# bodono/scs-python

Measured on AMD Instinct MI355X. Metric: ADMM iters/sec (random LP+SOC cone program, indirect CG linsys, AA lookback 10), higher is better.
Workload: dtype f64; 1 GPU; target_lp_soc: m=2000000 n=1000000 nnz=19999909 cone={'l': 1000000, 'q': '100000x10'} seed=5(+rank); one independent instance per GPU; world_size_seen=1

## Files before the change

### include/scs_hip.h

```cpp
#ifndef SCS_HIP_H_GUARD
#define SCS_HIP_H_GUARD

#include "scs_types.h"

#ifdef __cplusplus
extern "C" {
#endif

#define SCS_HIP_API __attribute__((visibility("default")))

typedef struct ScsHipWork ScsWork;


SCS_HIP_API ScsWork *scs_init(const ScsData *d, const ScsCone *k, const ScsSettings *stgs);

SCS_HIP_API scs_int scs_solve(ScsWork *w, ScsSolution *sol, ScsInfo *info, scs_int warm_start);

SCS_HIP_API scs_int scs_update(ScsWork *w, scs_float *b, scs_float *c);

SCS_HIP_API void scs_finish(ScsWork *w);

SCS_HIP_API void scs_set_default_settings(ScsSettings *stgs);

SCS_HIP_API const char *scs_version(void);
// ... 21 lines not shown

SCS_HIP_API int scs_hip_grad_matrix_sum(scs_int m, scs_int n, const scs_int *Ap, const scs_int *Ai, const scs_int *Pp, const scs_int *Pi, scs_int K,
                                        const scs_float *X, const scs_float *Y, const scs_float *DB, const scs_float *DC, scs_float *out_dA,
                                        scs_float *out_dP);

SCS_HIP_API int scs_hip_proj_cone_seq(scs_float *xs, const ScsCone *k, scs_int m, int dual, int count, scs_float *stats, int stats_cap);

SCS_HIP_API int scs_hip_kkt_solve(const ScsMatrix *A, const ScsMatrix *P, const scs_float *diag_r, scs_float *rhs,
                      scs_float tol, scs_int *cg_iters);

SCS_HIP_API int scs_hip_kkt_solve_dense(const ScsMatrix *A, const ScsMatrix *P, const scs_float *diag_r, scs_float *rhs);

SCS_HIP_API ScsWork *scs_hip_init_linsys(const ScsData *d, const ScsCone *k, const ScsSettings *stgs, int linsys);
SCS_HIP_API int scs_hip_linsys_kind(const ScsWork *w);

SCS_HIP_API int scs_hip_normalize(ScsMatrix *A, ScsMatrix *P, scs_float *b, scs_float *c, const ScsCone *k,
                      scs_float *D, scs_float *E, scs_float *sigma);

SCS_HIP_API double scs_hip_copy_bandwidth(size_t bytes, int reps);

SCS_HIP_API void scs_hip_set_profiling(ScsWork *w, int on);
SCS_HIP_API void scs_hip_kernel_times(const ScsWork *w, double *out);
SCS_HIP_API int scs_hip_solution_to_device(ScsWork *w, scs_float *x_dev, scs_float *y_dev, scs_float *s_dev);

SCS_HIP_API scs_int scs_hip_update_device(ScsWork *w, const scs_float *b_dev, const scs_float *c_dev);
SCS_HIP_API scs_int scs_hip_solve_device(ScsWork *w, scs_float *x_dev, scs_float *y_dev, scs_float *s_dev, ScsInfo *info, scs_int warm_start);
SCS_HIP_API scs_int scs_hip_solve_batch_device(ScsWork **w, scs_float **x_dev, scs_float **y_dev, scs_float **s_dev, ScsInfo **info,
                                               scs_int count, scs_int warm_start);
SCS_HIP_API scs_int scs_hip_update_matrix(ScsWork *w, const scs_float *Ax, const scs_float *Px);
SCS_HIP_API scs_int scs_hip_update_matrix_device(ScsWork *w, const scs_float *Ax_dev, const scs_float *Px_dev);
typedef struct {
  scs_float tol;
  scs_int max_iters;
} ScsHipDiffOpts;
typedef struct {
  scs_int iters;
  scs_float residual, normal_residual;
  scs_int stop;
  scs_float time_ms;
} ScsHipDiffInfo;
SCS_HIP_API scs_int scs_hip_adjoint_device(ScsWork *w, const scs_float *gx_dev, const scs_float *gy_dev, const scs_float *gs_dev,
                                           scs_float *db_dev, scs_float *dc_dev, scs_float *dAx_dev, scs_float *dPx_dev,
                                           const ScsHipDiffOpts *opts, ScsHipDiffInfo *info);
SCS_HIP_API scs_int scs_hip_adjoint(ScsWork *w, const scs_float *gx, const scs_float *gy, const scs_float *gs, scs_float *db, scs_float *dc,
                                    scs_float *dAx, scs_float *dPx, const ScsHipDiffOpts *opts, ScsHipDiffInfo *info);
SCS_HIP_API scs_int scs_hip_derivative_device(ScsWork *w, const scs_float *db_dev, const scs_float *dc_dev, scs_float *dx_dev,
// ... 96 lines not shown
```

### scs-python_amd/csrc/loop.hpp

```cpp
#pragma once
static void fill_nan(double *p, long nelem) {
  for (long i = 0; i < nelem; ++i) p[i] = NAN;
}

struct InterruptListener {
  static std::atomic<int> &flag() { static std::atomic<int> f{0}; return f; }
  static void on_sigint(int) { flag().store(1, std::memory_order_relaxed); }
  static bool enabled() { static const bool on = [] { const char *e = getenv("SCS_HIP_CTRLC"); return !(e && e[0] == '0'); }(); return on; }
  static std::mutex &mtx() { static std::mutex m; return m; }
  static int &users() { static int u = 0; return u; }
  static struct sigaction &saved() { static struct sigaction sa; return sa; }
  InterruptListener() {
    if (!enabled()) return;
    std::lock_guard<std::mutex> g(mtx());
    if (users()++ == 0) {
      flag().store(0);
      struct sigaction sa;
      std::memset(&sa, 0, sizeof(sa));
      sa.sa_handler = on_sigint;
      sigemptyset(&sa.sa_mask);
      sa.sa_flags = SA_RESTART;
      sigaction(SIGINT, &sa, &saved());
    }
  }
  ~InterruptListener() {
    if (!enabled()) return;
    std::lock_guard<std::mutex> g(mtx());
    if (--users() == 0) {
      struct sigaction cur;
      if (sigaction(SIGINT, nullptr, &cur) == 0 && cur.sa_handler == on_sigint) sigaction(SIGINT, &saved(), nullptr);
    }
  }
  static bool interrupted() { return enabled() && flag().load(std::memory_order_relaxed) != 0; }
};

static scs_int solve_impl(ScsHipWork *w, ScsSolution *sol, ScsInfo *info, scs_int warm_start, bool dev_io = false) {
  std::lock_guard<std::mutex> lock(w->mtx);
  InterruptListener ctrlc;
  HIP_CHECK(hipSetDevice(w->device));
  ScsHipWork::ScratchTurn turn(w);
  const int n = w->n, m = w->m;
  const long l = w->l;
  hipStream_t s = w->stream;
  w->finish_pending_setup();
  const double t_start = now_ms();
  w->begin_solve(sol, info, warm_start, dev_io);
  double t_lin = 0, t_cone = 0, t_acc = 0;
  FILE *csv = nullptr;
  if (!w->log_csv_filename.empty()) {
    csv = std::fopen(w->log_csv_filename.c_str(), "w");
    if (csv) std::fputs(kCsvHeader, csv);
  }
  const bool verbose = w->stgs.verbose != 0;
  if (verbose) {
    std::printf("------------------------------------------------------------------\n");
    std::printf("\t  scs-hip v%s - MI355X-native Splitting Conic Solver path\n", scs_version());
    std::printf("------------------------------------------------------------------\n");
    std::printf("problem:  variables n: %d, constraints m: %d\n", n, m);
    std::printf("cones: \t  z: %d, l: %d, box: %d, q: %zu, s: %zu, cs: %zu, ep: %d, ed: %d, p: %zu\n", w->cone.z, w->cone.l,
                w->cone.bsize, w->cone.q.size(), w->cone.s.size(), w->cone.cs.size(), w->cone.ep, w->cone.ed,
                w->cone.p.size());
    if (w->cone.has_spectral())
      std::printf("\t  d: %zu, nuc: %zu, ell1: %zu, sl: %zu\n", w->cone.d.size(), w->cone.nuc_m.size(), w->cone.ell1.size(),
                  w->cone.sl_n.size());
    std::printf("settings: eps_abs: %.1e, eps_rel: %.1e, eps_infeas: %.1e\n\t  alpha: %.2f, scale: %.2e, adaptive_scale: %d\n"
                "\t  max_iters: %d, normalize: %d, rho_x: %.2e\n\t  acceleration_lookback: %d, acceleration_interval: %d\n",
                w->stgs.eps_abs, w->stgs.eps_rel, w->stgs.eps_infeas, w->stgs.alpha, w->scale, w->stgs.adaptive_scale,
                w->stgs.max_iters, w->stgs.normalize, w->stgs.rho_x, w->stgs.acceleration_lookback,
                w->stgs.acceleration_interval);
// ... 78 lines not shown
      w->populate_residuals(i);
      std::printf("%6d|%9.2e|%9.2e|%9.2e|%9.2e|%9.2e|%9.2e\n", i, w->r.res_pri, w->r.res_dual, w->r.gap,
                  0.5 * (w->r.pobj + w->r.dobj), w->scale, (now_ms() - t_start) / 1e3);
      std::fflush(stdout);
    }
    if (w->stgs.adaptive_scale && check && i == w->r.last_iter) w->update_scale(i);
    w->enqueue_v_update();
    if (csv) w->log_csv_row(csv, i, now_ms() - t_start);
    if (aa_now) {
      t = now_ms();
      w->aa_safeguard();
      t_acc += now_ms() - t;
    }
  }
  if (csv) std::fclose(csv);
  if (w->debug_pipe()) {
    std::fprintf(stderr, "[scs-hip] iterations %d, run-ahead stalls %d, CG steps of the last 8 solves:", i, w->pipe_stalls);
    for (int v : w->cg_hist) std::fprintf(stderr, " %d", v);
    std::fprintf(stderr, "\n");
  }
  w->finish_solve(sol, info, i, t_start, t_lin, t_cone, t_acc, false, dev_io);
  std::vector<double> foot;
  ScsSolution foot_sol{nullptr, nullptr, nullptr};
  if (verbose && dev_io) {
    foot.resize(2 * (size_t)m);
    foot_sol.y = foot.data();
    foot_sol.s = foot.data() + m;
    w->soly.download(foot_sol.y, m, s);
    w->sols.download(foot_sol.s, m, s);
    HIP_CHECK(hipStreamSynchronize(s));
    sol = &foot_sol;
  }
  if (verbose) {
    std::printf("------------------------------------------------------------------\n");
    std::printf("status:  %s\ntimings: total: %.2es = setup: %.2es + solve: %.2es\n\t lin-sys: %.2es, cones: %.2es, accel: %.2es\n",
                info->status, (info->setup_time + info->solve_time) / 1e3, info->setup_time / 1e3, info->solve_time / 1e3,
                t_lin / 1e3, t_cone / 1e3, t_acc / 1e3);
    std::printf("lin-sys: avg cg its: %.2f\n", info->iter > 0 ? (double)w->tot_cg_iters / (info->iter + 1) : 0.0);
    std::printf("------------------------------------------------------------------\n");
    switch (info->status_val) {
      case SCS_SOLVED:
      case SCS_SOLVED_INACCURATE: {
        double sy = 0., ns = 0., ny = 0.;
        for (int j = 0; j < m; ++j) { sy += sol->s[j] * sol->y[j]; ns += sol->s[j] * sol->s[j]; ny += sol->y[j] * sol->y[j]; }
        std::printf("cones: dist(s, K) = %.2e, dist(y, K*) = %.2e\n", w->cone_dist(sol->s, 0), w->cone_dist(sol->y, 1));
        std::printf("comp slack: s'y/|s||y| = %.2e, gap: |x'Px+c'x+b'y| = %.2e\n", safediv_pos(sy, std::sqrt(ns) * std::sqrt(ny)), info->gap);
        std::printf("pri res: |Ax+s-b| = %.2e, dua res: |Px+A'y+c| = %.2e\n", info->res_pri, info->res_dual);
// ... 21 lines not shown
```

### scs-python_amd/csrc/options.hpp

```cpp
#pragma once
#include <atomic>
#include <cstdlib>
#include <cstring>
#include <mutex>
#include <string>

extern char **environ;

namespace scship {

enum : unsigned { DBG_PIPE = 1u, DBG_GROUP = 2u, DBG_SETUP = 4u, DBG_TOL = 8u };

struct Options {
  bool pipeline = true;
  int pipe_chunk = 0;
  bool host_setup = false;
  bool lazy_setup = true;
  bool cs = true;
  long cs_min_nnz = 1L << 20;
  bool cs_split = true;
  bool slab = true;
  bool aa_gram = false;
  int psd_split = -1;
  int psd_mc = -1;
  bool psd_refine = true;
  bool psd_tol_adaptive = true;
  int spin_budget_log2 = 25;
  bool linsys_dense = false;
  unsigned debug = 0;

  bool psd_coop = false;
  bool cs_combine = false;
  int cs_rpt = 0, cs_split_a = 0, cs_split_at = 0;
  bool cs_peel = true, cs_virt = true;
// ... 13 lines not shown
      o.pipe_chunk = v >= 2 ? v : 0;
    }
    if (const char *e = getenv("SCS_HIP_SETUP")) o.host_setup = e[0] == 'h';
    o.lazy_setup = !is0(getenv("SCS_HIP_LAZY_SETUP"));
    if (const char *e = getenv("SCS_HIP_CS")) {
      const long v = atol(e);
      o.cs = !is0(e);
      if (v >= 2) o.cs_min_nnz = v;
    }
    o.cs_split = !is0(getenv("SCS_HIP_CS_SPLIT"));
    o.slab = !is0(getenv("SCS_HIP_SLAB"));
    if (const char *e = getenv("SCS_HIP_AA")) o.aa_gram = e[0] == 'g';
    if (const char *e = getenv("SCS_HIP_PSD_SPLIT")) o.psd_split = e[0] == '1' ? 1 : 0;
    if (const char *e = getenv("SCS_HIP_PSD_MC")) o.psd_mc = atoi(e);
    o.psd_refine = !is0(getenv("SCS_HIP_PSD_REFINE"));
    if (const char *e = getenv("SCS_HIP_PSD_TOL")) o.psd_tol_adaptive = e[0] != 'f';
    if (const char *e = getenv("SCS_HIP_SPIN_BUDGET_LOG2")) { const int v = atoi(e); o.spin_budget_log2 = v < 0 ? 0 : (v > 40 ? 40 : v); }
    if (const char *e = getenv("SCS_HIP_LINSYS")) o.linsys_dense = e[0] == 'd' || e[0] == 'D';
    if (const char *e = getenv("SCS_HIP_DEBUG")) {
      if (strstr(e, "pipe")) o.debug |= DBG_PIPE;
      if (strstr(e, "group")) o.debug |= DBG_GROUP;
      if (strstr(e, "setup")) o.debug |= DBG_SETUP;
      if (strstr(e, "tol")) o.debug |= DBG_TOL;
      if (strstr(e, "all")) o.debug = ~0u;
    }
#ifdef SCS_HIP_LABS
    auto pos_int = [](const char *name, int dflt) { const char *e = getenv(name); const int v = e ? atoi(e) : 0; return v > 0 ? v : dflt; };
    auto pos_dbl = [](const char *name, double dflt) { const char *e = getenv(name); const double v = e ? atof(e) : 0.; return v > 0. ? v : dflt; };
    o.psd_coop = is1(getenv("SCS_HIP_PSD_COOP"));
    o.cs_combine = is1(getenv("SCS_HIP_CS_COMBINE"));
    { const int v = pos_int("SCS_HIP_CS_RPT", 0); o.cs_rpt = (v == 1 || v == 2 || v == 4 || v == 8 || v == 16) ? v : 0; }
    o.cs_split_a = pos_int("SCS_HIP_CS_SPLIT_A", 0);
    o.cs_split_at = pos_int("SCS_HIP_CS_SPLIT_AT", 0);
    o.cs_peel = !is0(getenv("SCS_HIP_CS_PEEL"));
    o.cs_virt = !is0(getenv("SCS_HIP_CS_VIRT"));
    o.cg_fuse = !is0(getenv("SCS_HIP_CG_FUSE"));
    o.norm_fuse = !is0(getenv("SCS_HIP_NORM_FUSE"));
    o.soc_psd_fuse = !is0(getenv("SCS_HIP_SOC_PSD_FUSE"));
    o.psd_tol_k = pos_dbl("SCS_HIP_PSD_TOL_K", 1e-2);
    o.psd_la = !is0(getenv("SCS_HIP_PSD_LA"));
    o.psd_mc_nocheck = getenv("SCS_HIP_PSD_MC_NOCHECK") != nullptr;
    o.pool_poison = is1(getenv("SCS_HIP_POOL_POISON"));
    if (const char *e = getenv("SCS_HIP_SHARED_TILE")) o.shared_tile = e[0] != '0';
#endif
    return o;
  }
// ... 27 lines not shown
```

### scs-python_amd/csrc/scs_hip.hip

```cpp
#include <atomic>
#include <cstddef>
#include <chrono>
#include <csignal>
#include <functional>
#include <memory>
#include <mutex>
#include <thread>

#include "options.hpp"
#include "aa.hpp"
#include "common.hpp"
#include "cones.hpp"
#include "host_setup.hpp"
#include "normalize_dev.hpp"
#include "psd.hpp"
#include "spectral.hpp"
#include "dense.hpp"
#include "setup_dev.hpp"
#include "setup_cs_dev.hpp"
#include "spmv.hpp"
#include "vec.hpp"
#include "device_io.hpp"
#include "dproj.hpp"
#include "lsqr.hpp"

#include "runtime.hpp"
#include "device_csr.hpp"
#include "work.hpp"
#include "io.hpp"
#include "setup.hpp"
#include "loop.hpp"
#include "batch.hpp"
#include "matrix_update.hpp"
#include "perturb.hpp"
#include "diff.hpp"
#include "diff_batch.hpp"
#include "grad_shared.hpp"

static ScsCone short_cone(const ScsCone *k) {
  ScsCone c;
  std::memset(&c, 0, sizeof(c));
  if (k) std::memcpy(&c, k, offsetof(ScsCone, d));
  return c;
}

extern "C" {

ScsWork *scs_init(const ScsData *d, const ScsCone *k, const ScsSettings *stgs) {
  try {
// ... 28 lines not shown
}

ScsWork *scs_hip_init_linsys_spectral(const ScsData *d, const ScsCone *k, const ScsSettings *stgs, int linsys) {
  try {
    set_last_error("");
    return init_impl(d, k, stgs, linsys);
  } catch (const std::exception &e) {
    set_last_error(e.what());
    return nullptr;
  }
}
ScsWork *scs_hip_clone(ScsWork *w) {
  try {
    set_last_error("");
    return clone_impl(w);
  } catch (const std::exception &e) {
    set_last_error(e.what());
    return nullptr;
  }
}
int scs_hip_shares_matrix(const ScsWork *a, const ScsWork *b) { return a && b && a->mats == b->mats ? 1 : 0; }
int scs_hip_linsys_kind(const ScsWork *w) { return w ? (w->dense() ? 2 : 1) : 0; }

static void fill_failed(ScsHipWork *w, ScsSolution *sol, bool dev_io) {
  if (!dev_io) {
    fill_nan(sol->x, w->n);
    fill_nan(sol->y, w->m);
    fill_nan(sol->s, w->m);
    return;
  }
  if (hipSetDevice(w->device) != hipSuccess) return;
  const double *ptr[3] = {sol->x, sol->y, sol->s};
  const long len[3] = {w->n, w->m, w->m};
  for (int k = 0; k < 3; ++k)
    if (ptr[k]) hipLaunchKernelGGL(k_fill, dim3(vec_blocks(len[k])), dim3(kVecThreads), 0, w->stream, (double *)ptr[k], (double)NAN, len[k]);
  (void)hipStreamSynchronize(w->stream);
  (void)hipGetLastError();
}

static scs_int solve_entry(ScsWork *w, ScsSolution *sol, ScsInfo *info, scs_int warm_start, bool dev_io) {
  try {
    set_last_error("");
    const double scale_entry = w->scale;
    try {
      return solve_impl(w, sol, info, warm_start, dev_io);
    } catch (const SpinTimeout &) {
      ++g_spin_fallbacks;
      {
        std::lock_guard<std::mutex> lock(w->mtx);
        HIP_CHECK(hipSetDevice(w->device));
        w->spin_fallback(scale_entry);
      }
      return solve_impl(w, sol, info, warm_start, dev_io);
    }
  } catch (const std::exception &e) {
    set_last_error(e.what());
    info->status_val = SCS_FAILED;
    std::snprintf(info->status, sizeof(info->status), "failure");
    fill_failed(w, sol, dev_io);
    return SCS_FAILED;
  }
}

scs_int scs_solve(ScsWork *w, ScsSolution *sol, ScsInfo *info, scs_int warm_start) {
  if (!w || !sol || !info) return SCS_FAILED;
  return solve_entry(w, sol, info, warm_start, false);
}

static void check_device_vector(const void *p, int device, const char *who, const char *name) {
  hipPointerAttribute_t a;
  std::memset(&a, 0, sizeof(a));
  const hipError_t e = hipPointerGetAttributes(&a, p);
  if (e != hipSuccess) (void)hipGetLastError();
  if (e != hipSuccess || a.type != hipMemoryTypeDevice)
    throw std::runtime_error(std::string(who) + ": " + name + " is not a device address");
  if (a.device != device)
    throw std::runtime_error(std::string(who) + ": " + name + " lives on device " + std::to_string(a.device) + ", the workspace on device " +
                             std::to_string(device));
}
static void check_device_solution(const ScsHipWork *w, const double *x, const double *y, const double *s, scs_int warm_start, const char *who) {
  if (warm_start && (!x || !y || !s)) throw std::runtime_error(std::string(who) + ": a warm start needs x_dev, y_dev and s_dev");
  if (x) check_device_vector(x, w->device, who, "x_dev");
  if (y) check_device_vector(y, w->device, who, "y_dev");
  if (s) check_device_vector(s, w->device, who, "s_dev");
}

scs_int scs_hip_update_device(ScsWork *w, const scs_float *b_dev, const scs_float *c_dev) {
  if (!w) return -1;
  try {
// ... 2 lines not shown
    if (c_dev) check_device_vector(c_dev, w->device, "scs_hip_update_device", "c_dev");
    std::lock_guard<std::mutex> lock(w->mtx);
    HIP_CHECK(hipSetDevice(w->device));
    ScsHipWork::ScratchTurn turn(w);
    w->diff_mark_stale();
    w->update_device(b_dev, c_dev);
    return 0;
  } catch (const std::exception &e) {
    set_last_error(e.what());
    return -1;
  }
}

scs_int scs_hip_solve_device(ScsWork *w, scs_float *x_dev, scs_float *y_dev, scs_float *s_dev, ScsInfo *info, scs_int warm_start) {
  if (!w || !info) return -1;
  try {
    set_last_error("");
    check_device_solution(w, x_dev, y_dev, s_dev, warm_start, "scs_hip_solve_device");
  } catch (const std::exception &e) {
    set_last_error(e.what());
    return -1;
  }
  ScsSolution sol{x_dev, y_dev, s_dev};
  return solve_entry(w, &sol, info, warm_start, true);
}
int scs_hip_work_device(const ScsWork *w) { return w ? w->device : -1; }

static scs_int solve_one_group(ScsWork **works, ScsSolution **sols, ScsInfo **infos, const std::vector<int> &idx, scs_int warm_start,
                               std::string &err, bool dev_io, const Options &o) {
  if (idx.size() == 1) {
    const int i = idx[0];
    const scs_int st = solve_entry(works[i], sols[i], infos[i], warm_start, dev_io);
    if (st == SCS_FAILED) { err = scs_hip_last_error(); return -1; }
    return 0;
  }
  scs_int rc = 0;
  std::vector<std::unique_lock<std::mutex>> locks;
  std::vector<hipStream_t> saved;
  GroupSolve gs(o);
  for (int j : idx) {
    std::memset(infos[j], 0, sizeof(ScsInfo));
    infos[j]->status_val = SCS_UNFINISHED;
  }
  try {
    {
      std::vector<int> order(idx);
      std::sort(order.begin(), order.end(), [&](int a, int b) { return std::less<ScsHipWork *>()(works[a], works[b]); });
      for (int j : order) locks.emplace_back(works[j]->mtx);
    }
    HIP_CHECK(hipSetDevice(works[idx[0]]->device));
    gs.s = works[idx[0]]->stream;
    gs.dev_io = dev_io;
    for (int j : idx) {
      gs.W.push_back(works[j]); gs.sols.push_back(sols[j]); gs.infos.push_back(infos[j]);
      saved.push_back(works[j]->stream);
// ... 910 lines not shown
```

### scs-python_amd/csrc/work.hpp

```cpp
#pragma once
using namespace scship;

static void write_csv_row(FILE *f, int iter, const Residuals &r, double scale, const double *diffs, double aa_norm,
                          double time_s);

struct SpinTimeout : std::runtime_error {
  using std::runtime_error::runtime_error;
};
static std::atomic<long> g_spin_fallbacks{0};
struct SpinChain {
  std::mutex mu;
  int users = 0;
  hipEvent_t last = nullptr;
  hipStream_t last_stream = nullptr;
};
static SpinChain &spin_chain(int device) {
  static SpinChain c[64];
  return c[device & 63];
}

struct MatrixSet {
  const Options &opt;
  explicit MatrixSet(const Options &o) : opt(o) {}
  std::shared_ptr<Arena> home;
// ... 68 lines not shown

  DeviceCsr &At = mats->At;
  DeviceCsr &Ar = mats->Ar;
  DeviceCsr &Pf = mats->Pf;
  DevBuf<double> &Pdiag = mats->Pdiag;
  DevBuf<double> &D = mats->D, &E = mats->E;

  DevBuf<double> v, v_prev, u, ut, rsk, g, h, diag_r, Dinv, Einv;
  DevBuf<double> cg_b, cg_p, cg_r, cg_Gp, cg_M, tmp_m, ws, px;
  DevBuf<double> part, part2, sc, out;
  DevBuf<double> part_v;
  bool v_norm_fresh = false;
  DevBuf<int> fl;
  DevBuf<double> solx, soly, sols;
  bool sol_on_device = false;
  int diff_state = 0, last_status_val = 0;
  void diff_mark_stale() { if (diff_state == 1) diff_state = 3; }
  DiffScratch diff;
  DevBuf<double> b_raw, c_raw;
  DevBuf<unsigned> io_ticket;
  bool b_raw_fresh = false, c_raw_fresh = false, b_host_stale = false, c_host_stale = false;
  double *sol_pin = nullptr;
  bool sol_pin_refused = false;
  hipEvent_t sol_ev[3] = {nullptr, nullptr, nullptr};
  static constexpr size_t kSolMirrorMin = (size_t)1 << 20;
  static void spread_memcpy(void *dst, const void *src, size_t bytes) {
    const int nt = bytes >= ((size_t)8 << 20) ? 4 : 1;
    if (nt == 1) { std::memcpy(dst, src, bytes); return; }
    const size_t part = (bytes / nt + 4095) & ~(size_t)4095;
    std::thread th[3];
    for (int t = 1; t < nt; ++t) {
      const size_t o = std::min(bytes, part * t), c = std::min(bytes - o, part);
      th[t - 1] = std::thread([=] { if (c) std::memcpy((char *)dst + o, (const char *)src + o, c); });
    }
    std::memcpy(dst, src, std::min(bytes, part));
    for (int t = 1; t < nt; ++t) th[t - 1].join();
  }
  void ensure_solution_mirror() {
    const size_t bytes = sizeof(double) * ((size_t)n + 2 * (size_t)m);
    if (sol_pin || sol_pin_refused || bytes < kSolMirrorMin) return;
    if (hipHostMalloc((void **)&sol_pin, bytes, hipHostMallocDefault) != hipSuccess) {
      (void)hipGetLastError();
      sol_pin = nullptr;
      sol_pin_refused = true;
      return;
    }
    for (auto &e : sol_ev) HIP_CHECK(hipEventCreateWithFlags(&e, hipEventDisableTiming));
  }
  void download_solution(ScsSolution *sol) {
    ensure_solution_mirror();
    if (!sol_pin) {
      solx.download(sol->x, n, stream);
      soly.download(sol->y, m, stream);
      sols.download(sol->s, m, stream);
      HIP_CHECK(hipStreamSynchronize(stream));
      return;
    }
    double *hx = sol_pin, *hy = sol_pin + n, *hs = sol_pin + n + m;
    solx.download(hx, n, stream); HIP_CHECK(hipEventRecord(sol_ev[0], stream));
    soly.download(hy, m, stream); HIP_CHECK(hipEventRecord(sol_ev[1], stream));
    sols.download(hs, m, stream); HIP_CHECK(hipEventRecord(sol_ev[2], stream));
    HIP_CHECK(hipEventSynchronize(sol_ev[0])); spread_memcpy(sol->x, hx, sizeof(double) * n);
    HIP_CHECK(hipEventSynchronize(sol_ev[1])); spread_memcpy(sol->y, hy, sizeof(double) * m);
    HIP_CHECK(hipEventSynchronize(sol_ev[2])); spread_memcpy(sol->s, hs, sizeof(double) * m);
    HIP_CHECK(hipStreamSynchronize(stream));
  }
  int part_len = 0;

  DevBuf<int> soc_off, soc_dim, soc_big;
  int n_soc = 0, n_soc_big = 0, soc_G = 64;
  DevBuf<double> pow_a, box_bl, box_bu;
  DevBuf<double> box_bl_orig, box_bu_orig, box_parts;
  DevBuf<unsigned> cg_ticket;
  DevBuf<unsigned> box_ticket;
  DevBuf<int> psd_off, psd_order;
  DevBuf<long> psd_woff;
  std::vector<long> psd_woff_h;
  std::vector<int> psd_order_h;
  DevBuf<double> psd_scratch;
  int n_psd = 0, n_psd_big = 0;
  static constexpr int kPsdSplitRounds = 2;
  bool psd_split = false;
  int psd_max_np = 0, psd_max_tiles = 0;
  DevBuf<int> cs_off, cs_order, cs_poff, cs_porder;
  DevBuf<long> cs_soff, cs_woff;
  DevBuf<double> cs_stage;
  int n_cs = 0, n_cs_big = 0;
  DevBuf<int> spec_meta;
// ... 244 lines not shown
```

### scs-python_amd/scs/_scs_hip.py

```python
import collections
import contextlib
import functools
import ctypes as C
import importlib.util
import os
import threading
import warnings

import numpy as np

_HERE = os.path.dirname(os.path.abspath(__file__))
_LIB_NAME = "libscs_hip.so"

c_int, c_dbl = C.c_int, C.c_double
_PI, _PD = C.POINTER(c_int), C.POINTER(c_dbl)


class _ScsMatrix(C.Structure):
    _fields_ = [("x", _PD), ("i", _PI), ("p", _PI), ("m", c_int), ("n", c_int)]


class _ScsData(C.Structure):
    _fields_ = [("m", c_int), ("n", c_int), ("A", C.POINTER(_ScsMatrix)),
                ("P", C.POINTER(_ScsMatrix)), ("b", _PD), ("c", _PD)]
# ... 134 lines not shown
    lib.scs_hip_spmv.restype = c_int
    lib.scs_hip_spmv.argtypes = [C.POINTER(_ScsMatrix), _PD, _PD, c_int]
    lib.scs_hip_cs_layout_host_spmv.restype = c_int
    lib.scs_hip_cs_layout_host_spmv.argtypes = [C.POINTER(_ScsMatrix), _PD, _PD, c_int, c_int, c_int]
    lib.scs_hip_spmv_bench.restype = c_dbl
    lib.scs_hip_spmv_bench.argtypes = [C.POINTER(_ScsMatrix), c_int, c_int]
    lib.scs_hip_proj_cone.restype = c_int
    lib.scs_hip_proj_cone.argtypes = [_PD, C.POINTER(_ScsCone), c_int, c_int]
    lib.scs_hip_proj_cone_seq.restype = c_int
    lib.scs_hip_proj_cone_seq.argtypes = [_PD, C.POINTER(_ScsCone), c_int, c_int, c_int, _PD, c_int]
    lib.scs_hip_kkt_solve.restype = c_int
    lib.scs_hip_kkt_solve.argtypes = [C.POINTER(_ScsMatrix), C.POINTER(_ScsMatrix), _PD, _PD, c_dbl, _PI]
    lib.scs_hip_normalize.restype = c_int
    lib.scs_hip_normalize.argtypes = [C.POINTER(_ScsMatrix), C.POINTER(_ScsMatrix), _PD, _PD,
                                      C.POINTER(_ScsCone), _PD, _PD, _PD]
    lib.scs_hip_normalize_spectral.restype = c_int
    lib.scs_hip_normalize_spectral.argtypes = lib.scs_hip_normalize.argtypes
    lib.scs_hip_set_profiling.restype = None
    lib.scs_hip_set_profiling.argtypes = [C.c_void_p, c_int]
    lib.scs_hip_kernel_times.restype = None
    lib.scs_hip_kernel_times.argtypes = [C.c_void_p, _PD]
    lib.scs_hip_solution_to_device.restype = c_int
    lib.scs_hip_solution_to_device.argtypes = [C.c_void_p, C.c_void_p, C.c_void_p, C.c_void_p]
    lib.scs_hip_update_device.restype = c_int
    lib.scs_hip_update_device.argtypes = [C.c_void_p, C.c_void_p, C.c_void_p]
    lib.scs_hip_update_matrix.restype = c_int
    lib.scs_hip_update_matrix.argtypes = [C.c_void_p, C.c_void_p, C.c_void_p]
    lib.scs_hip_update_matrix_device.restype = c_int
    lib.scs_hip_update_matrix_device.argtypes = [C.c_void_p, C.c_void_p, C.c_void_p]
    lib.scs_hip_solve_device.restype = c_int
    lib.scs_hip_solve_device.argtypes = [C.c_void_p, C.c_void_p, C.c_void_p, C.c_void_p, C.POINTER(_ScsInfo), c_int]
    lib.scs_hip_solve_batch_device.restype = c_int
    lib.scs_hip_solve_batch_device.argtypes = [C.POINTER(C.c_void_p), C.POINTER(C.c_void_p), C.POINTER(C.c_void_p), C.POINTER(C.c_void_p),
                                               C.POINTER(C.POINTER(_ScsInfo)), c_int, c_int]
    for name in ("scs_hip_adjoint", "scs_hip_adjoint_device"):
        fn = getattr(lib, name)
        fn.restype = c_int
        fn.argtypes = [C.c_void_p] + [C.c_void_p] * 7 + [C.POINTER(_ScsHipDiffOpts), C.POINTER(_ScsHipDiffInfo)]
    for name in ("scs_hip_derivative", "scs_hip_derivative_device"):
        fn = getattr(lib, name)
        fn.restype = c_int
        fn.argtypes = [C.c_void_p] + [C.c_void_p] * 5 + [C.POINTER(_ScsHipDiffOpts), C.POINTER(_ScsHipDiffInfo)]
    for name in ("scs_hip_derivative_full", "scs_hip_derivative_full_device"):
        fn = getattr(lib, name)
        fn.restype = c_int
        fn.argtypes = [C.c_void_p] + [C.c_void_p] * 7 + [C.POINTER(_ScsHipDiffOpts), C.POINTER(_ScsHipDiffInfo)]
# ... 152 lines not shown
def _as_c_double(name, v):
    if isinstance(v, (str, bytes)) or v is None:
        raise TypeError("must be real number, not %s" % type(v).__name__)
    try:
        return float(v)
    except (TypeError, ValueError):
        raise TypeError("must be real number, not %s" % type(v).__name__)


def _as_bool(name, v):
    if not isinstance(v, (bool, np.bool_)):
        raise TypeError("argument '%s' must be bool, not %s" % (name, type(v).__name__))
    return 1 if v else 0


def _as_filename(name, v):
    if v is None:
        return None
    if isinstance(v, str):
        return v.encode()
    raise TypeError("argument '%s' must be str or None, not %s" % (name, type(v).__name__))


_INT_SETTINGS = ("max_iters", "acceleration_lookback", "acceleration_interval", "acceleration_type_1")
_FLOAT_SETTINGS = ("scale", "eps_abs", "eps_rel", "eps_infeas", "alpha", "rho_x", "time_limit_secs",
                   "acceleration_regularization", "acceleration_relaxation")
_BOOL_SETTINGS = ("verbose", "normalize", "adaptive_scale")
_FILE_SETTINGS = ("write_data_filename", "log_csv_filename")


def _cone_err(key):
    return ValueError("Invalid value for cone field '%s'" % key)


def _cone_pos_int(cone, key):
    if key not in cone:
        return 0
    v = cone[key]
    if isinstance(v, (bool, np.bool_)) or not isinstance(v, (int, np.integer)):
        raise _cone_err(key)
    v = int(v)
    if v < 0 or v >= 2 ** 31:
        raise _cone_err(key)
    return v


# ... 192 lines not shown
        k = _ScsCone(z, lcone, _pd(bu), _pd(bl), (bu.size + 1) if bu.size > 0 else 0,
                     _pi(q), q.size, _pi(s), s.size, _pi(cs), cs.size, ep, ed, _pd(p), p.size)
        _set_spectral(k, spec)
        if self._LINSYS:
            work = _lib.scs_hip_init_linsys_spectral(C.byref(d), C.byref(k), C.byref(st), self._LINSYS)
        else:
            work = _lib.scs_init_spectral(C.byref(d), C.byref(k), C.byref(st))
        if not work:
            self._init_error = last_error()
            raise ValueError("ScsWork allocation error!" + (" (%s)" % self._init_error if self._init_error else ""))
        self._work = work
        self._pattern = {"A": (Apc, Aic), "P": (Ppc, Pic) if have_P else None}

    def _blank(self):
        self._work = None
        self._lock = threading.Lock()
        self._fn_keep = []
        self._many = []
        self._pattern = None

    def _shape(self, m, n):
        self.m, self.n = m, n
        self._x, self._y, self._s = np.zeros(n), np.zeros(m), np.zeros(m)

    def _warm(self, name, dst, src):
        if not isinstance(src, np.ndarray) or not np.issubdtype(src.dtype, np.floating) or src.ndim != 1:
            raise ValueError("Unable to parse %s warm-start" % name)
        if src.shape[0] != dst.shape[0]:
            raise ValueError("Unable to parse %s warm-start" % name)
        dst[:] = src

    def solve(self, warm_start=True, x=None, y=None, s=None):
        if not isinstance(warm_start, (bool, np.bool_)):
            raise TypeError("argument 1 must be bool, not %s" % type(warm_start).__name__)
        with self._lock:
            if not self._work:
                raise ValueError("Workspace not initialized!")
            if warm_start:
                if x is not None:
                    self._warm("x", self._x, x)
                if y is not None:
                    self._warm("y", self._y, y)
                if s is not None:
                    self._warm("s", self._s, s)
            sol = _ScsSolution(_pd(self._x), _pd(self._y), _pd(self._s))
            info = _ScsInfo()
            _lib.scs_solve(self._work, C.byref(sol), C.byref(info), 1 if warm_start else 0)
            xo, yo, so = self._x.copy(), self._y.copy(), self._s.copy()
        info_dict = _info_dict(info)
        return {"x": xo, "y": yo, "s": so, "info": info_dict}

    def update(self, b=None, c=None):
        cc = bc = None
        if c is not None:
            if not isinstance(c, np.ndarray) or not np.issubdtype(c.dtype, np.floating) or c.ndim != 1:
                raise TypeError("c_new must be a 1-D numpy array of floats")
            if c.shape[0] != self.n:
                raise ValueError("c_new has incompatible dimension with A")
            cc = np.array(c, dtype=np.float64, order="C", copy=True)
        if b is not None:
            if not isinstance(b, np.ndarray) or not np.issubdtype(b.dtype, np.floating) or b.ndim != 1:
                raise TypeError("b_new must be a 1-D numpy array of floats")
            if b.shape[0] != self.m:
                raise ValueError("b_new has incompatible dimension with A")
            bc = np.array(b, dtype=np.float64, order="C", copy=True)
        with self._lock:
            if not self._work:
                raise ValueError("Workspace not initialized!")
            _lib.scs_update(self._work, _pd(bc) if bc is not None else None, _pd(cc) if cc is not None else None)
        return None

    def _finish_many(self):
        pool, self._many = self._many, []
        for sv in pool:
            sv.__del__()

    def _update_matrix_call(self, fn, ap, pp):
        self._finish_many()
        with self._lock:
            if not self._work:
                raise ValueError("Workspace not initialized!")
            rc = fn(self._work, ap, pp)
            err = last_error() if rc != 0 else ""
        if rc != 0:
            raise ValueError("libscs_hip: " + err)
        return None

    def update_matrix(self, A=None, P=None):
        if not self._work:
            raise ValueError("Workspace not initialized!")
        av = _matrix_values("A", A, self._pattern["A"]) if A is not None else None
        pv = _matrix_values("P", P, self._pattern["P"]) if P is not None else None
        if av is None and pv is None:
            return None
        return self._update_matrix_call(_lib.scs_hip_update_matrix, _pd(av) if av is not None else None, _pd(pv) if pv is not None else None)

    def update_matrix_device(self, A=None, P=None):
        dev = self._device_index()
        if P is not None and self._pattern["P"] is None:
            raise ValueError("P given, but the solver was created without P")
        ap = _device_vec("A", A, int(self._pattern["A"][1].shape[0]), dev) if A is not None else None
        pp = _device_vec("P", P, int(self._pattern["P"][1].shape[0]), dev) if P is not None else None
        if ap is None and pp is None:
            return None
# ... 13 lines not shown
        new._work = work
        new._pattern = self._pattern
        return new

    def shares_matrix(self, other):
        if not isinstance(other, SCS) or not self._work or not other._work:
            return False
        return bool(_lib.scs_hip_shares_matrix(self._work, other._work))

    def solve_many(self, b=None, c=None, warm_start=False, x=None, y=None, s=None):
        K, rows = _many_args(self.m, self.n, b, c, warm_start, x, y, s)
        if not self._work:
            raise ValueError("Workspace not initialized!")
        pool = self._many
        while len(pool) < K - 1:
            pool.append(self.clone())
        members = [self] + pool[:K - 1]
        for i, sv in enumerate(members):
            bi, ci = rows["b"][i] if b is not None else None, rows["c"][i] if c is not None else None
            if bi is not None or ci is not None:
                sv.update(bi, ci)
            if warm_start:
                with sv._lock:
                    for name, dst in (("x", sv._x), ("y", sv._y), ("s", sv._s)):
                        if rows[name] is not None:
                            sv._warm(name, dst, rows[name][i])
        return solve_batch(members, bool(warm_start))

    def _device_index(self):
        if not self._work:
            raise ValueError("Workspace not initialized!")
        return int(_lib.scs_hip_work_device(self._work))

    def update_device(self, b=None, c=None):
        dev = self._device_index()
        bp = _device_vec("b_new", b, self.m, dev) if b is not None else None
        cp = _device_vec("c_new", c, self.n, dev) if c is not None else None
        _sync_torch_stream(dev)
        with self._lock:
            if not self._work:
                raise ValueError("Workspace not initialized!")
            rc = _lib.scs_hip_update_device(self._work, bp, cp)
            err = last_error() if rc != 0 else ""
        if rc != 0:
            raise RuntimeError("libscs_hip: " + err)
        return None

    def _previous_to_device(self, ptrs):
        got = _lib.scs_hip_solution_to_device(self._work, ptrs.get("x"), ptrs.get("y"), ptrs.get("s")) == 0
        return got

    def solve_device(self, warm_start=False, x=None, y=None, s=None):
        if not isinstance(warm_start, (bool, np.bool_)):
            raise TypeError("argument 1 must be bool, not %s" % type(warm_start).__name__)
        dev = self._device_index()
        given = {}
        if warm_start:
            for name, t, length in (("x", x, self.n), ("y", y, self.m), ("s", s, self.m)):
                if t is not None:
                    _device_vec(name, t, length, dev)
                    given[name] = t
        import torch
        tdev = torch.device("cuda", dev)
        out = {"x": torch.empty(self.n, dtype=torch.float64, device=tdev), "y": torch.empty(self.m, dtype=torch.float64, device=tdev),
               "s": torch.empty(self.m, dtype=torch.float64, device=tdev)}
        with self._lock:
            if not self._work:
                raise ValueError("Workspace not initialized!")
            if warm_start:
                for name, t in given.items():
                    out[name].copy_(t)
                missing = {name: out[name].data_ptr() for name in out if name not in given}
                if missing:
                    for name in missing:
                        out[name].zero_()
                    _sync_torch_stream(dev)
                    self._previous_to_device(missing)
            _sync_torch_stream(dev)
            info = _ScsInfo()
            rc = _lib.scs_hip_solve_device(self._work, out["x"].data_ptr(), out["y"].data_ptr(), out["s"].data_ptr(), C.byref(info),
                                           1 if warm_start else 0)
            err = last_error() if rc == -1 else ""
        if rc == -1 and info.status_val == 0:
            raise RuntimeError("libscs_hip: " + err)
        out["info"] = _info_dict(info)
        return out

    def solve_many_device(self, b=None, c=None, warm_start=False, x=None, y=None, s=None):
        dev = self._device_index()
        K, rows = _many_device_args(self.m, self.n, dev, b, c, warm_start, x, y, s)
        pool = self._many
        while len(pool) < K - 1:
            pool.append(self.clone())
        members = [self] + pool[:K - 1]
        for i, sv in enumerate(members):
            bi, ci = rows["b"][i] if b is not None else None, rows["c"][i] if c is not None else None
            if bi is not None or ci is not None:
                sv.update_device(bi, ci)
        import torch
        tdev = torch.device("cuda", dev)
        out = {"x": torch.empty((K, self.n), dtype=torch.float64, device=tdev), "y": torch.empty((K, self.m), dtype=torch.float64, device=tdev),
               "s": torch.empty((K, self.m), dtype=torch.float64, device=tdev)}
        with _locked(members) as works:
            if warm_start:
                missing = [name for name in ("x", "y", "s") if rows[name] is None]
                for name in ("x", "y", "s"):
                    if rows[name] is not None:
                        out[name].copy_(rows[name])
                    else:
                        out[name].zero_()
                _sync_torch_stream(dev)
                if missing:
                    for i, sv in enumerate(members):
                        sv._previous_to_device({name: out[name][i].data_ptr() for name in missing})
            _sync_torch_stream(dev)
            infos = [_ScsInfo() for _ in members]
            ptrs = {name: (C.c_void_p * K)(*[out[name][i].data_ptr() for i in range(K)]) for name in ("x", "y", "s")}
            infp = (C.POINTER(_ScsInfo) * K)(*[C.pointer(io) for io in infos])
            rc = _lib.scs_hip_solve_batch_device(works, ptrs["x"], ptrs["y"], ptrs["s"], infp, K, 1 if warm_start else 0)
            err = last_error() if rc != 0 else ""
        out["info"] = [_info_dict(io) for io in infos]
        if rc != 0 and any(o["status_val"] == 0 for o in out["info"]):
            raise RuntimeError("libscs_hip: " + err)
        return out

    def _diff_call(self, fn, ptrs, opts):
# ... 343 lines not shown
def _batch_solvers(solvers, who):
    solvers = list(solvers)
    for sv in solvers:
        if not isinstance(sv, SCS):
            raise TypeError("%s expects scs._scs_hip.SCS objects" % who)
    if len(set(id(sv) for sv in solvers)) != len(solvers):
        raise ValueError("%s: a solver appears twice" % who)
    return solvers


def solve_batch(solvers, warm_start=False):
    if not isinstance(warm_start, (bool, np.bool_)):
        raise TypeError("argument 2 must be bool, not %s" % type(warm_start).__name__)
    solvers = list(solvers)
    if not solvers:
        return []
    if len(set(id(sv) for sv in solvers)) != len(solvers):
        raise ValueError("solve_batch: a solver appears twice")
    for sv in solvers:
        if not isinstance(sv, SCS):
            raise TypeError("solve_batch expects scs._scs_hip.SCS objects")
    with _locked(solvers) as works:
        cnt = len(solvers)
        sols = [_ScsSolution(_pd(sv._x), _pd(sv._y), _pd(sv._s)) for sv in solvers]
        infos = [_ScsInfo() for _ in solvers]
        solp = (C.POINTER(_ScsSolution) * cnt)(*[C.pointer(so) for so in sols])
        infp = (C.POINTER(_ScsInfo) * cnt)(*[C.pointer(io) for io in infos])
        rc = _lib.scs_hip_solve_batch(works, solp, infp, cnt, 1 if warm_start else 0)
        err = last_error() if rc != 0 else ""
        out = [{"x": sv._x.copy(), "y": sv._y.copy(), "s": sv._s.copy(), "info": _info_dict(io)}
               for sv, io in zip(solvers, infos)]
    if rc != 0 and any(o["info"]["status_val"] == 0 for o in out):
        raise RuntimeError("libscs_hip: " + err)
    return out


def _plan_call(solvers, plan):
    with _locked(solvers) as works:
        out = (c_int * len(solvers))()
        rc = plan(works, len(solvers), out)
        err = last_error() if rc < 0 else ""
    if rc < 0:
        raise RuntimeError("libscs_hip: " + err)
    return [int(v) for v in out]


def batch_plan(solvers):
    solvers = list(solvers)
    if not solvers:
        return []
    if len(set(id(sv) for sv in solvers)) != len(solvers):
        raise ValueError("batch_plan: a solver appears twice")
    for sv in solvers:
        if not isinstance(sv, SCS):
# ... 442 lines not shown
```

Before: 788.1 ADMM iters/s.

## Solve into fresh output arrays and pipeline chunked solution download

The Python solve now passes separate warm-start and output buffers to a new solve_to entry point. This removes the host-side copies of x, y and s after each solve, and the solver's own host mirror is refreshed lazily only when a later call needs it. The pinned-buffer download is split into 4 MB chunks, each with its own event, so host memcpy by a small thread pool overlaps the remaining DMA. This adds extra state tracking (_host_stale) and more code paths, and the change only touches the end-of-solve transfer rather than the per-iteration ADMM work.

New measurement: 792.6 ADMM iters/s (median of 5 runs). About the same (+0.6%).

```diff
diff --git a/include/scs_hip.h b/include/scs_hip.h
--- a/include/scs_hip.h
+++ b/include/scs_hip.h
@@ -67,6 +67,9 @@
 SCS_HIP_API void scs_hip_set_profiling(ScsWork *w, int on);
 SCS_HIP_API void scs_hip_kernel_times(const ScsWork *w, double *out);
 SCS_HIP_API int scs_hip_solution_to_device(ScsWork *w, scs_float *x_dev, scs_float *y_dev, scs_float *s_dev);
+
+SCS_HIP_API scs_int scs_hip_solve_to(ScsWork *w, const ScsSolution *warm, ScsSolution *out, ScsInfo *info, scs_int warm_start);
+SCS_HIP_API int scs_hip_solution_to_host(ScsWork *w, scs_float *x, scs_float *y, scs_float *s);
 
 SCS_HIP_API scs_int scs_hip_update_device(ScsWork *w, const scs_float *b_dev, const scs_float *c_dev);
 SCS_HIP_API scs_int scs_hip_solve_device(ScsWork *w, scs_float *x_dev, scs_float *y_dev, scs_float *s_dev, ScsInfo *info, scs_int warm_start);
diff --git a/scs-python_amd/csrc/host_copy.hpp b/scs-python_amd/csrc/host_copy.hpp
--- /dev/null
+++ b/scs-python_amd/csrc/host_copy.hpp
@@ -0,0 +1,103 @@
+#pragma once
+#include <algorithm>
+#include <condition_variable>
+#include <cstddef>
+#include <cstring>
+#include <deque>
+#include <mutex>
+#include <thread>
+#include <vector>
+
+namespace scship {
+
+constexpr size_t kSolChunkBytes = (size_t)4 << 20;
+constexpr size_t kCopyPieceAlign = 4096;
+constexpr int kCopyThreadsMax = 4;
+constexpr size_t kCopyThreadsMin = (size_t)8 << 20;
+
+struct CopyChunk {
+  size_t off, bytes;
+};
+inline std::vector<CopyChunk> chunk_plan(size_t bytes, size_t chunk) {
+  std::vector<CopyChunk> plan;
+  for (size_t off = 0; off < bytes; off += chunk) plan.push_back(CopyChunk{off, std::min(chunk, bytes - off)});
+  return plan;
+}
+inline int copy_threads_for(size_t total) { return total >= kCopyThreadsMin ? kCopyThreadsMax : 1; }
+
+class CopyQueue {
+ public:
+  explicit CopyQueue(int threads) : nthreads_(std::max(1, std::min(threads, kCopyThreadsMax))) {
+    try {
+      for (int t = 1; t < nthreads_; ++t) helpers_.emplace_back([this] { serve(true); });
+    } catch (...) {
+      finish();
+      throw;
+    }
+  }
+  CopyQueue(const CopyQueue &) = delete;
+  CopyQueue &operator=(const CopyQueue &) = delete;
+  ~CopyQueue() { finish(); }
+
+  void push(void *dst, const void *src, size_t bytes) {
+    if (!bytes) return;
+    if (nthreads_ == 1) {
+      std::memcpy(dst, src, bytes);
+      return;
+    }
+    const size_t piece = std::max(kCopyPieceAlign, (bytes / nthreads_ + kCopyPieceAlign - 1) / kCopyPieceAlign * kCopyPieceAlign);
+    {
+      std::lock_guard<std::mutex> lk(mu_);
+      for (size_t off = 0; off < bytes; off += piece)
+        q_.push_back(Piece{(char *)dst + off, (const char *)src + off, std::min(piece, bytes - off)});
+    }
+    cv_.notify_all();
+  }
+  void finish() {
+    if (closed_) return;
+    {
+      std::lock_guard<std::mutex> lk(mu_);
+      closed_ = true;
+    }
+    cv_.notify_all();
+    serve(false);
+    for (std::thread &t : helpers_) t.join();
+    helpers_.clear();
+  }
+
+ private:
+  struct Piece {
+    char *dst;
+    const char *src;
+    size_t bytes;
+  };
+  void serve(bool until_closed) {
+    for (;;) {
+      Piece p;
+      {
+        std::unique_lock<std::mutex> lk(mu_);
+        if (until_closed) cv_.wait(lk, [this] { return !q_.empty() || closed_; });
+        if (q_.empty()) return;
+        p = q_.front();
+        q_.pop_front();
+      }
+      std::memcpy(p.dst, p.src, p.bytes);
+    }
+  }
+  const int nthreads_;
+  bool closed_ = false;
+  std::mutex mu_;
+  std::condition_variable cv_;
+  std::deque<Piece> q_;
+  std::vector<std::thread> helpers_;
+};
+
+template <class Landed>
+inline void copy_out_chunks(CopyQueue &q, void *dst, const void *src, const std::vector<CopyChunk> &plan, Landed &&landed) {
+  for (size_t i = 0; i < plan.size(); ++i) {
+    landed(i);
+    q.push((char *)dst + plan[i].off, (const char *)src + plan[i].off, plan[i].bytes);
+  }
+}
+
+}
diff --git a/scs-python_amd/csrc/loop.hpp b/scs-python_amd/csrc/loop.hpp
--- a/scs-python_amd/csrc/loop.hpp
+++ b/scs-python_amd/csrc/loop.hpp
@@ -34,7 +34,7 @@
   static bool interrupted() { return enabled() && flag().load(std::memory_order_relaxed) != 0; }
 };
 
-static scs_int solve_impl(ScsHipWork *w, ScsSolution *sol, ScsInfo *info, scs_int warm_start, bool dev_io = false) {
+static scs_int solve_impl(ScsHipWork *w, const ScsSolution *warm, const ScsSolution *sol, ScsInfo *info, scs_int warm_start, bool dev_io = false) {
   std::lock_guard<std::mutex> lock(w->mtx);
   InterruptListener ctrlc;
   HIP_CHECK(hipSetDevice(w->device));
@@ -44,7 +44,7 @@
   hipStream_t s = w->stream;
   w->finish_pending_setup();
   const double t_start = now_ms();
-  w->begin_solve(sol, info, warm_start, dev_io);
+  w->begin_solve(warm, info, warm_start, dev_io);
   double t_lin = 0, t_cone = 0, t_acc = 0;
   FILE *csv = nullptr;
   if (!w->log_csv_filename.empty()) {
@@ -169,7 +169,7 @@
   w->finish_solve(sol, info, i, t_start, t_lin, t_cone, t_acc, false, dev_io);
   std::vector<double> foot;
   ScsSolution foot_sol{nullptr, nullptr, nullptr};
-  if (verbose && dev_io) {
+  if (verbose && (dev_io || !sol->y || !sol->s)) {
     foot.resize(2 * (size_t)m);
     foot_sol.y = foot.data();
     foot_sol.s = foot.data() + m;
diff --git a/scs-python_amd/csrc/options.hpp b/scs-python_amd/csrc/options.hpp
--- a/scs-python_amd/csrc/options.hpp
+++ b/scs-python_amd/csrc/options.hpp
@@ -9,7 +9,7 @@
 
 namespace scship {
 
-enum : unsigned { DBG_PIPE = 1u, DBG_GROUP = 2u, DBG_SETUP = 4u, DBG_TOL = 8u };
+enum : unsigned { DBG_PIPE = 1u, DBG_GROUP = 2u, DBG_SETUP = 4u, DBG_TOL = 8u, DBG_ENDS = 16u };
 
 struct Options {
   bool pipeline = true;
@@ -69,6 +69,7 @@
       if (strstr(e, "group")) o.debug |= DBG_GROUP;
       if (strstr(e, "setup")) o.debug |= DBG_SETUP;
       if (strstr(e, "tol")) o.debug |= DBG_TOL;
+      if (strstr(e, "ends")) o.debug |= DBG_ENDS;
       if (strstr(e, "all")) o.debug = ~0u;
     }
 #ifdef SCS_HIP_LABS
diff --git a/scs-python_amd/csrc/scs_hip.hip b/scs-python_amd/csrc/scs_hip.hip
--- a/scs-python_amd/csrc/scs_hip.hip
+++ b/scs-python_amd/csrc/scs_hip.hip
@@ -25,6 +25,7 @@
 #include "lsqr.hpp"
 
 #include "runtime.hpp"
+#include "host_copy.hpp"
 #include "device_csr.hpp"
 #include "work.hpp"
 #include "io.hpp"
@@ -99,11 +100,11 @@
 int scs_hip_shares_matrix(const ScsWork *a, const ScsWork *b) { return a && b && a->mats == b->mats ? 1 : 0; }
 int scs_hip_linsys_kind(const ScsWork *w) { return w ? (w->dense() ? 2 : 1) : 0; }
 
-static void fill_failed(ScsHipWork *w, ScsSolution *sol, bool dev_io) {
+static void fill_failed(ScsHipWork *w, const ScsSolution *sol, bool dev_io) {
   if (!dev_io) {
-    fill_nan(sol->x, w->n);
-    fill_nan(sol->y, w->m);
-    fill_nan(sol->s, w->m);
+    if (sol->x) fill_nan(sol->x, w->n);
+    if (sol->y) fill_nan(sol->y, w->m);
+    if (sol->s) fill_nan(sol->s, w->m);
     return;
   }
   if (hipSetDevice(w->device) != hipSuccess) return;
@@ -115,12 +116,12 @@
   (void)hipGetLastError();
 }
 
-static scs_int solve_entry(ScsWork *w, ScsSolution *sol, ScsInfo *info, scs_int warm_start, bool dev_io) {
+static scs_int solve_entry(ScsWork *w, const ScsSolution *warm, const ScsSolution *sol, ScsInfo *info, scs_int warm_start, bool dev_io) {
   try {
     set_last_error("");
     const double scale_entry = w->scale;
     try {
-      return solve_impl(w, sol, info, warm_start, dev_io);
+      return solve_impl(w, warm, sol, info, warm_start, dev_io);
     } catch (const SpinTimeout &) {
       ++g_spin_fallbacks;
       {
@@ -128,7 +129,7 @@
         HIP_CHECK(hipSetDevice(w->device));
         w->spin_fallback(scale_entry);
       }
-      return solve_impl(w, sol, info, warm_start, dev_io);
+      return solve_impl(w, warm, sol, info, warm_start, dev_io);
     }
   } catch (const std::exception &e) {
     set_last_error(e.what());
@@ -141,7 +142,33 @@
 
 scs_int scs_solve(ScsWork *w, ScsSolution *sol, ScsInfo *info, scs_int warm_start) {
   if (!w || !sol || !info) return SCS_FAILED;
-  return solve_entry(w, sol, info, warm_start, false);
+  return solve_entry(w, sol, sol, info, warm_start, false);
+}
+
+scs_int scs_hip_solve_to(ScsWork *w, const ScsSolution *warm, ScsSolution *out, ScsInfo *info, scs_int warm_start) {
+  if (!w || !out || !info) return SCS_FAILED;
+  return solve_entry(w, warm, out, info, warm_start, false);
+}
+
+int scs_hip_solution_to_host(ScsWork *w, scs_float *x, scs_float *y, scs_float *s) {
+  if (!w) return -1;
+  try {
+    set_last_error("");
+    std::lock_guard<std::mutex> lock(w->mtx);
+    if (!w->sol_on_device) {
+      if (x) std::fill(x, x + w->n, 0.0);
+      if (y) std::fill(y, y + w->m, 0.0);
+      if (s) std::fill(s, s + w->m, 0.0);
+      return 1;
+    }
+    HIP_CHECK(hipSetDevice(w->device));
+    const ScsSolution out{x, y, s};
+    w->download_solution(&out);
+    return 0;
+  } catch (const std::exception &e) {
+    set_last_error(e.what());
+    return -1;
+  }
 }
 
 static void check_device_vector(const void *p, int device, const char *who, const char *name) {
@@ -190,7 +217,7 @@
     return -1;
   }
   ScsSolution sol{x_dev, y_dev, s_dev};
-  return solve_entry(w, &sol, info, warm_start, true);
+  return solve_entry(w, &sol, &sol, info, warm_start, true);
 }
 int scs_hip_work_device(const ScsWork *w) { return w ? w->device : -1; }
 
@@ -198,7 +225,7 @@
                                std::string &err, bool dev_io, const Options &o) {
   if (idx.size() == 1) {
     const int i = idx[0];
-    const scs_int st = solve_entry(works[i], sols[i], infos[i], warm_start, dev_io);
+    const scs_int st = solve_entry(works[i], sols[i], sols[i], infos[i], warm_start, dev_io);
     if (st == SCS_FAILED) { err = scs_hip_last_error(); return -1; }
     return 0;
   }
diff --git a/scs-python_amd/csrc/work.hpp b/scs-python_amd/csrc/work.hpp
--- a/scs-python_amd/csrc/work.hpp
+++ b/scs-python_amd/csrc/work.hpp
@@ -114,20 +114,8 @@
   bool b_raw_fresh = false, c_raw_fresh = false, b_host_stale = false, c_host_stale = false;
   double *sol_pin = nullptr;
   bool sol_pin_refused = false;
-  hipEvent_t sol_ev[3] = {nullptr, nullptr, nullptr};
+  std::vector<hipEvent_t> sol_ev;
   static constexpr size_t kSolMirrorMin = (size_t)1 << 20;
-  static void spread_memcpy(void *dst, const void *src, size_t bytes) {
-    const int nt = bytes >= ((size_t)8 << 20) ? 4 : 1;
-    if (nt == 1) { std::memcpy(dst, src, bytes); return; }
-    const size_t part = (bytes / nt + 4095) & ~(size_t)4095;
-    std::thread th[3];
-    for (int t = 1; t < nt; ++t) {
-      const size_t o = std::min(bytes, part * t), c = std::min(bytes - o, part);
-      th[t - 1] = std::thread([=] { if (c) std::memcpy((char *)dst + o, (const char *)src + o, c); });
-    }
-    std::memcpy(dst, src, std::min(bytes, part));
-    for (int t = 1; t < nt; ++t) th[t - 1].join();
-  }
   void ensure_solution_mirror() {
     const size_t bytes = sizeof(double) * ((size_t)n + 2 * (size_t)m);
     if (sol_pin || sol_pin_refused || bytes < kSolMirrorMin) return;
@@ -135,27 +123,57 @@
       (void)hipGetLastError();
       sol_pin = nullptr;
       sol_pin_refused = true;
-      return;
-    }
-    for (auto &e : sol_ev) HIP_CHECK(hipEventCreateWithFlags(&e, hipEventDisableTiming));
-  }
-  void download_solution(ScsSolution *sol) {
+    }
+  }
+  void download_solution(const ScsSolution *out) {
     ensure_solution_mirror();
+    double *const dst[3] = {out->x, out->y, out->s};
+    const double *const src[3] = {solx.p, soly.p, sols.p};
+    const size_t bytes[3] = {sizeof(double) * (size_t)n, sizeof(double) * (size_t)m, sizeof(double) * (size_t)m};
     if (!sol_pin) {
-      solx.download(sol->x, n, stream);
-      soly.download(sol->y, m, stream);
-      sols.download(sol->s, m, stream);
+      for (int k = 0; k < 3; ++k)
+        if (dst[k] && bytes[k]) HIP_CHECK(hipMemcpyAsync(dst[k], src[k], bytes[k], hipMemcpyDeviceToHost, stream));
       HIP_CHECK(hipStreamSynchronize(stream));
       return;
     }
-    double *hx = sol_pin, *hy = sol_pin + n, *hs = sol_pin + n + m;
-    solx.download(hx, n, stream); HIP_CHECK(hipEventRecord(sol_ev[0], stream));
-    soly.download(hy, m, stream); HIP_CHECK(hipEventRecord(sol_ev[1], stream));
-    sols.download(hs, m, stream); HIP_CHECK(hipEventRecord(sol_ev[2], stream));
-    HIP_CHECK(hipEventSynchronize(sol_ev[0])); spread_memcpy(sol->x, hx, sizeof(double) * n);
-    HIP_CHECK(hipEventSynchronize(sol_ev[1])); spread_memcpy(sol->y, hy, sizeof(double) * m);
-    HIP_CHECK(hipEventSynchronize(sol_ev[2])); spread_memcpy(sol->s, hs, sizeof(double) * m);
+    const double t0 = now_ms();
+    char *const pin[3] = {(char *)sol_pin, (char *)(sol_pin + n), (char *)(sol_pin + n + m)};
+    std::vector<CopyChunk> plan[3];
+    size_t total = 0, nev = 0;
+    for (int k = 0; k < 3; ++k)
+      if (dst[k]) {
+        plan[k] = chunk_plan(bytes[k], kSolChunkBytes);
+        total += bytes[k];
+        nev += plan[k].size();
+      }
+    while (sol_ev.size() < nev) {
+      hipEvent_t e = nullptr;
+      HIP_CHECK(hipEventCreateWithFlags(&e, hipEventDisableTiming));
+      sol_ev.push_back(e);
+    }
+    size_t queued = 0;
+    for (int k = 0; k < 3; ++k)
+      for (const CopyChunk &c : plan[k]) {
+        HIP_CHECK(hipMemcpyAsync(pin[k] + c.off, (const char *)src[k] + c.off, c.bytes, hipMemcpyDeviceToHost, stream));
+        HIP_CHECK(hipEventRecord(sol_ev[queued++], stream));
+      }
+    double t_last = t0;
+    {
+      CopyQueue q(copy_threads_for(total));
+      size_t landed = 0;
+      for (int k = 0; k < 3; ++k)
+        copy_out_chunks(q, dst[k], pin[k], plan[k], [&](size_t) {
+          HIP_CHECK(hipEventSynchronize(sol_ev[landed++]));
+          if (landed == nev) t_last = now_ms();
+        });
+      q.finish();
+    }
     HIP_CHECK(hipStreamSynchronize(stream));
+    if (opt.debug & DBG_ENDS) {
+      const double t1 = now_ms();
+      std::fprintf(stderr, "[scs-hip] download_solution: %zu bytes in %zu chunks, %.3f ms until the last DMA event (%.1f GB/s), %.3f ms after it\n",
+                   total, nev, t_last - t0, (double)total / 1e6 / std::max(t_last - t0, 1e-6), t1 - t_last);
+    }
   }
   int part_len = 0;
 
diff --git a/scs-python_amd/scs/_scs_hip.py b/scs-python_amd/scs/_scs_hip.py
--- a/scs-python_amd/scs/_scs_hip.py
+++ b/scs-python_amd/scs/_scs_hip.py
@@ -180,6 +180,10 @@
     lib.scs_hip_kernel_times.argtypes = [C.c_void_p, _PD]
     lib.scs_hip_solution_to_device.restype = c_int
     lib.scs_hip_solution_to_device.argtypes = [C.c_void_p, C.c_void_p, C.c_void_p, C.c_void_p]
+    lib.scs_hip_solve_to.restype = c_int
+    lib.scs_hip_solve_to.argtypes = [C.c_void_p, C.POINTER(_ScsSolution), C.POINTER(_ScsSolution), C.POINTER(_ScsInfo), c_int]
+    lib.scs_hip_solution_to_host.restype = c_int
+    lib.scs_hip_solution_to_host.argtypes = [C.c_void_p, _PD, _PD, _PD]
     lib.scs_hip_update_device.restype = c_int
     lib.scs_hip_update_device.argtypes = [C.c_void_p, C.c_void_p, C.c_void_p]
     lib.scs_hip_update_matrix.restype = c_int
@@ -378,6 +382,7 @@
     raise TypeError("argument '%s' must be str or None, not %s" % (name, type(v).__name__))
 
 
+_SCS_FAILED = -4
 _INT_SETTINGS = ("max_iters", "acceleration_lookback", "acceleration_interval", "acceleration_type_1")
 _FLOAT_SETTINGS = ("scale", "eps_abs", "eps_rel", "eps_infeas", "alpha", "rho_x", "time_limit_secs",
                    "acceleration_regularization", "acceleration_relaxation")
@@ -616,12 +621,23 @@
     def _shape(self, m, n):
         self.m, self.n = m, n
         self._x, self._y, self._s = np.zeros(n), np.zeros(m), np.zeros(m)
-
-    def _warm(self, name, dst, src):
+        self._host_stale = True
+
+    def _refresh_host(self):
+        if self._host_stale:
+            if _lib.scs_hip_solution_to_host(self._work, _pd(self._x), _pd(self._y), _pd(self._s)) < 0:
+                raise RuntimeError("libscs_hip: " + last_error())
+            self._host_stale = False
+
+    @staticmethod
+    def _warm_check(name, length, src):
         if not isinstance(src, np.ndarray) or not np.issubdtype(src.dtype, np.floating) or src.ndim != 1:
             raise ValueError("Unable to parse %s warm-start" % name)
-        if src.shape[0] != dst.shape[0]:
+        if src.shape[0] != length:
             raise ValueError("Unable to parse %s warm-start" % name)
+
+    def _warm(self, name, dst, src):
+        self._warm_check(name, dst.shape[0], src)
         dst[:] = src
 
     def solve(self, warm_start=True, x=None, y=None, s=None):
@@ -630,17 +646,24 @@
         with self._lock:
             if not self._work:
                 raise ValueError("Workspace not initialized!")
-            if warm_start:
-                if x is not None:
-                    self._warm("x", self._x, x)
-                if y is not None:
-                    self._warm("y", self._y, y)
-                if s is not None:
-                    self._warm("s", self._s, s)
-            sol = _ScsSolution(_pd(self._x), _pd(self._y), _pd(self._s))
+            warm = []
+            for name, src, mine in (("x", x, self._x), ("y", y, self._y), ("s", s, self._s)):
+                if warm_start and src is not None:
+                    self._warm_check(name, mine.shape[0], src)
+                    warm.append(np.ascontiguousarray(src, dtype=np.float64))
+                else:
+                    warm.append(mine if warm_start and not self._host_stale else None)
+            wsol = _ScsSolution(*[_pd(a) if a is not None else None for a in warm])
+            xo, yo, so = np.empty(self.n), np.empty(self.m), np.empty(self.m)
+            sol = _ScsSolution(_pd(xo), _pd(yo), _pd(so))
             info = _ScsInfo()
-            _lib.scs_solve(self._work, C.byref(sol), C.byref(info), 1 if warm_start else 0)
-            xo, yo, so = self._x.copy(), self._y.copy(), self._s.copy()
+            _lib.scs_hip_solve_to(self._work, C.byref(wsol), C.byref(sol), C.byref(info), 1 if warm_start else 0)
+            if info.status_val == _SCS_FAILED:
+                for a in (self._x, self._y, self._s):
+                    a.fill(np.nan)
+                self._host_stale = False
+            else:
+                self._host_stale = True
         info_dict = _info_dict(info)
         return {"x": xo, "y": yo, "s": so, "info": info_dict}
 
@@ -674,6 +697,7 @@
         with self._lock:
             if not self._work:
                 raise ValueError("Workspace not initialized!")
+            self._refresh_host()
             rc = fn(self._work, ap, pp)
             err = last_error() if rc != 0 else ""
         if rc != 0:
@@ -733,6 +757,9 @@
                 sv.update(bi, ci)
             if warm_start:
                 with sv._lock:
+                    if not sv._work:
+                        raise ValueError("Workspace not initialized!")
+                    sv._refresh_host()
                     for name, dst in (("x", sv._x), ("y", sv._y), ("s", sv._s)):
                         if rows[name] is not None:
                             sv._warm(name, dst, rows[name][i])
@@ -778,6 +805,7 @@
         with self._lock:
             if not self._work:
                 raise ValueError("Workspace not initialized!")
+            self._refresh_host()
             if warm_start:
                 for name, t in given.items():
                     out[name].copy_(t)
@@ -813,6 +841,8 @@
         out = {"x": torch.empty((K, self.n), dtype=torch.float64, device=tdev), "y": torch.empty((K, self.m), dtype=torch.float64, device=tdev),
                "s": torch.empty((K, self.m), dtype=torch.float64, device=tdev)}
         with _locked(members) as works:
+            for sv in members:
+                sv._refresh_host()
             if warm_start:
                 missing = [name for name in ("x", "y", "s") if rows[name] is None]
                 for name in ("x", "y", "s"):
@@ -1202,6 +1232,9 @@
             raise TypeError("solve_batch expects scs._scs_hip.SCS objects")
     with _locked(solvers) as works:
         cnt = len(solvers)
+        if warm_start:
+            for sv in solvers:
+                sv._refresh_host()
         sols = [_ScsSolution(_pd(sv._x), _pd(sv._y), _pd(sv._s)) for sv in solvers]
         infos = [_ScsInfo() for _ in solvers]
         solp = (C.POINTER(_ScsSolution) * cnt)(*[C.pointer(so) for so in sols])
@@ -1210,6 +1243,9 @@
         err = last_error() if rc != 0 else ""
         out = [{"x": sv._x.copy(), "y": sv._y.copy(), "s": sv._s.copy(), "info": _info_dict(io)}
                for sv, io in zip(solvers, infos)]
+        for sv, io in zip(solvers, infos):
+            if io.status_val != 0:
+                sv._host_stale = False
     if rc != 0 and any(o["info"]["status_val"] == 0 for o in out):
         raise RuntimeError("libscs_hip: " + err)
     return out
```
